# re-ovo/wgpu-path-tracing

Hardware: AMD Instinct MI355X
Metric: Msamples/s (rays x bounces / s) (higher is better)
Workload: dtype f32

## Files before the change

### wgpu-path-tracing_amd/csrc/pipeline.hip

```cpp
#include "pt_device.h"
#include "pt_math.h"

namespace {

constexpr int BLOCK = 256;

PT_DEV void camera_ray(const ptmi_camera &cam, uint32_t x, uint32_t y, uint32_t frame, v3 &org, v3 &dir,
                       uint32_t &rng) {
    rng = rng_seed(x, y, frame);
    float jx = rng_f(rng), jy = rng_f(rng);
    float px = (float)x + jx, py = (float)y + jy;
    float uvx = (px / (float)cam.width) * 2.0f - 1.0f;
    float uvy = (py / (float)cam.height) * 2.0f - 1.0f;
    float th = tan1(cam.fov * 0.5f);
    v3 fw = mk3(cam.forward[0], cam.forward[1], cam.forward[2]);
    v3 rt = mk3(cam.right[0], cam.right[1], cam.right[2]);
    v3 up = mk3(cam.up[0], cam.up[1], cam.up[2]);
    v3 pos = mk3(cam.position[0], cam.position[1], cam.position[2]);
    v3 a = scale3(scale3(scale3(rt, uvx), th), cam.aspect);
    v3 b = scale3(scale3(up, uvy), th);
    dir = normalize3(add3(add3(fw, a), b));
    org = pos;
    if (cam.aperture > 0.0f) {
        v3 focal = madd3(dir, cam.focus_distance, pos);
// ... 68 lines not shown
    __shared__ uint32_t wsum[TILE_WAVES], wssum[TILE_WAVES];
    const uint32_t count = *count_ptr;
    const uint32_t nwords = (count + 63u) >> 6;
    if (blockIdx.x == 0 && threadIdx.x == 0) {
        atomicAdd(&stats[0], (unsigned long long)count); atomicAdd(&stats[8 + bounce], (unsigned long long)count);
    }
    if (blockIdx.x * TILE_WORDS >= nwords) return;
    const uint32_t w = blockIdx.x * TILE_WORDS + threadIdx.x;
    uint32_t c = 0, sc = 0;
    if (w < nwords) { c = (uint32_t)__popcll(alive[w]); if (shadow) sc = (uint32_t)__popcll(shadow[w]); }
    for (int off = 32; off > 0; off >>= 1) { c += __shfl_down(c, off); sc += __shfl_down(sc, off); }
    if ((threadIdx.x & 63u) == 0u) { wsum[threadIdx.x >> 6] = c; wssum[threadIdx.x >> 6] = sc; }
    __syncthreads();
    if (threadIdx.x == 0) {
        uint32_t t = 0, ts = 0;
        for (int i = 0; i < TILE_WAVES; i++) { t += wsum[i]; ts += wssum[i]; }
        tile_sums[blockIdx.x] = t;
        shadow_tile_sums[blockIdx.x] = ts;
        if (ts) { atomicAdd(&stats[1], (unsigned long long)ts); atomicAdd(&stats[2], (unsigned long long)ts); }
    }
}

template <bool PACKED>
PT_DEV void scatter_tile(uint32_t tile, const uint32_t *__restrict__ count_ptr, const uint32_t *__restrict__ queue,
                         const uint64_t *__restrict__ alive, const uint32_t *__restrict__ tile_sums,
                         uint32_t *__restrict__ next_queue, uint32_t *__restrict__ next_count) {
    __shared__ uint32_t wtot[TILE_WAVES];
    __shared__ uint32_t tile_base;
    const uint32_t count = *count_ptr;
    const uint32_t nwords = (count + 63u) >> 6;
    const uint32_t ntiles = (nwords + TILE_WORDS - 1) / TILE_WORDS;
    if (tile >= ntiles) {
        if (ntiles == 0 && tile == 0 && threadIdx.x == 0) *next_count = 0;
        return;
    }
    const uint32_t lane = threadIdx.x & 63u, wave = threadIdx.x >> 6;
    uint32_t pre = 0;
    for (uint32_t t = threadIdx.x; t < tile; t += TILE_WORDS) pre += tile_sums[t];
    for (int off = 32; off > 0; off >>= 1) pre += __shfl_down(pre, off);
    if (lane == 0) wtot[wave] = pre;
    __syncthreads();
    if (threadIdx.x == 0) { uint32_t t = 0; for (int i = 0; i < TILE_WAVES; i++) t += wtot[i]; tile_base = t; }
    __syncthreads();
    const uint32_t base0 = tile_base;
    __syncthreads();
    const uint32_t w = tile * TILE_WORDS + threadIdx.x;
    const uint64_t m = w < nwords ? alive[w] : 0ull;
    const uint32_t c = (uint32_t)__popcll(m);
    uint32_t inc = c;
    for (int off = 1; off < 64; off <<= 1) { uint32_t v = __shfl_up(inc, off); if (lane >= (uint32_t)off) inc += v; }
    if (lane == 63u) wtot[wave] = inc;
    __syncthreads();
    uint32_t wbase = 0;
    for (uint32_t i = 0; i < wave; i++) wbase += wtot[i];
    const uint32_t my_off = base0 + wbase + inc - c;
    if (tile == ntiles - 1 && threadIdx.x == TILE_WORDS - 1) *next_count = my_off + c;
    const uint32_t mlo = (uint32_t)m, mhi = (uint32_t)(m >> 32);
    const uint32_t w0 = tile * TILE_WORDS + wave * 64u;
    for (uint32_t j = 0; j < 64u; j++) {
        const uint32_t jlo = __shfl(mlo, (int)j), jhi = __shfl(mhi, (int)j), jbase = __shfl(my_off, (int)j);
        const uint64_t jm = ((uint64_t)jhi << 32) | jlo;
        if (jm == 0ull) continue;
        if ((jm >> lane) & 1ull) {
            const uint32_t below = (uint32_t)__popcll(jm & ((1ull << lane) - 1ull));
            const uint32_t slot = (w0 + j) * 64u + lane;
            next_queue[jbase + below] = PACKED ? (w0 + j) * 64u + below : queue ? queue[slot] : slot;
        }
    }
}

__global__ __launch_bounds__(TILE_WORDS) void k_scatter(const uint32_t *__restrict__ count_ptr,
                                                        const uint32_t *__restrict__ queue,
                                                        const uint64_t *__restrict__ alive,
                                                        const uint32_t *__restrict__ tile_sums,
                                                        uint32_t *__restrict__ next_queue,
                                                        uint32_t *__restrict__ next_count) {
    scatter_tile<false>(blockIdx.x, count_ptr, queue, alive, tile_sums, next_queue, next_count);
}
__global__ __launch_bounds__(TILE_WORDS) void k_scatter_packed(const uint32_t *__restrict__ count_ptr,
                                                               const uint64_t *__restrict__ shadow,
                                                               const uint32_t *__restrict__ shadow_sums,
                                                               uint32_t *__restrict__ shadow_queue,
                                                               uint32_t *__restrict__ shadow_count) {
    scatter_tile<true>(blockIdx.x, count_ptr, nullptr, shadow, shadow_sums, shadow_queue, shadow_count);
}
__global__ __launch_bounds__(TILE_WORDS) void k_scatter2(uint32_t tiles, const uint32_t *__restrict__ count_ptr,
                                                         const uint32_t *__restrict__ queue,
                                                         const uint64_t *__restrict__ alive, const uint64_t *__restrict__ shadow,
                                                         const uint32_t *__restrict__ tile_sums, const uint32_t *__restrict__ shadow_sums,
                                                         uint32_t *__restrict__ next_queue, uint32_t *__restrict__ next_count,
                                                         uint32_t *__restrict__ shadow_queue, uint32_t *__restrict__ shadow_count) {
    if (blockIdx.x < tiles) scatter_tile<false>(blockIdx.x, count_ptr, queue, alive, tile_sums, next_queue, next_count);
    else scatter_tile<true>(blockIdx.x - tiles, count_ptr, nullptr, shadow, shadow_sums, shadow_queue, shadow_count);
}

__global__ __launch_bounds__(BLOCK) void k_repack(const uint32_t *__restrict__ count_ptr, const uint32_t *__restrict__ queue,
                                                  DevPaths from, DevPaths to, uint32_t *__restrict__ pid) {
    const uint32_t n = *count_ptr;
    for (uint32_t j = blockIdx.x * BLOCK + threadIdx.x; j < n; j += gridDim.x * BLOCK) {
        const uint32_t q = queue[j];
        const float4 o = ld_stream(&from.O[q]), d = ld_stream(&from.D[q]);
        const float2 c = ld_stream(&from.C[q]);
        st_stream(&to.O[j], o); st_stream(&to.D[j], d); st_stream(&to.C[j], c);
        pid[j] = q;
    }
}

template <int N>
PT_DEV void fold(float (&acc)[N], const float (&x)[N], uint32_t frame) {
    if (frame > 0u) {
        const float t = 1.0f / (float)(frame + 1u);
        for (int i = 0; i < N; i++) acc[i] = mix1(acc[i], x[i], t);
    } else {
        for (int i = 0; i < N; i++) acc[i] = x[i];
    }
}
PT_DEV rgb_sc ld_clamped(const float *__restrict__ L, uint32_t l_stride, size_t p) {
    rgb_sc l;
    if (l_stride == 4u) { const float4 v = reinterpret_cast<const float4 *>(L)[p]; l = rgb_sc{v.x, v.y, v.z}; }
    else l = reinterpret_cast<const rgb_sc *>(L)[p];
    return rgb_sc{min1(l.x, 2.5f), min1(l.y, 2.5f), min1(l.z, 2.5f)};
}

template <class Pixels>
PT_DEV void fold_radiance(const Pixels &px, uint32_t n_frames, const float *__restrict__ L, uint32_t l_stride, float4 *__restrict__ out) {
    const uint32_t n = px.entries();
    for (uint32_t j = blockIdx.x * BLOCK + threadIdx.x; j < n; j += gridDim.x * BLOCK) {
        const size_t oi = px.band.frame_pixel(px.pixel(j));
// ... 110 lines not shown
        const uint64_t word = __ballot(active);
        if ((threadIdx.x & 63u) == 0u) ballot[pix >> 6] = word;
    }
}

__global__ __launch_bounds__(TILE_WORDS) void k_ad_tile_sums(const uint32_t *__restrict__ count_ptr, const uint64_t *__restrict__ ballot,
                                                             uint32_t *__restrict__ tile_sums) {
    __shared__ uint32_t wsum[TILE_WAVES];
    const uint32_t nwords = (*count_ptr + 63u) >> 6;
    const uint32_t w = blockIdx.x * TILE_WORDS + threadIdx.x;
    uint32_t c = w < nwords ? (uint32_t)__popcll(ballot[w]) : 0u;
    for (int off = 32; off > 0; off >>= 1) c += __shfl_down(c, off);
    if ((threadIdx.x & 63u) == 0u) wsum[threadIdx.x >> 6] = c;
    __syncthreads();
    if (threadIdx.x == 0) {
        uint32_t t = 0;
        for (int i = 0; i < TILE_WAVES; i++) t += wsum[i];
        tile_sums[blockIdx.x] = t;
    }
}
__global__ __launch_bounds__(TILE_WORDS) void k_ad_scatter(const uint32_t *__restrict__ count_ptr, const uint64_t *__restrict__ ballot,
                                                           const uint32_t *__restrict__ tile_sums, uint32_t *__restrict__ list,
                                                           uint32_t *__restrict__ n_active) {
    scatter_tile<false>(blockIdx.x, count_ptr, nullptr, ballot, tile_sums, list, n_active);
}

__global__ __launch_bounds__(BLOCK) void k_ad_raygen(ptmi_camera cam, DevBand band, const uint32_t *__restrict__ list,
                                                     const uint32_t *__restrict__ n_active, uint32_t n_frames,
                                                     const float4 *__restrict__ mom, DevPaths P, uint32_t *__restrict__ count_out,
                                                     unsigned long long *__restrict__ traced) {
    if (blockIdx.x == 0 && threadIdx.x == 0) atomicAdd(&traced[0], (unsigned long long)(*n_active * n_frames));
    raygen(cam, ListedPixels{band, list, n_active, mom}, n_frames, P, count_out);
}
__global__ __launch_bounds__(BLOCK) void k_ad_accumulate(DevBand band, const uint32_t *__restrict__ list, const uint32_t *__restrict__ n_active,
                                                         uint32_t n_frames, const float4 *__restrict__ mom, const float *__restrict__ L,
                                                         uint32_t l_stride, float4 *__restrict__ out) {
    fold_radiance(ListedPixels{band, list, n_active, mom}, n_frames, L, l_stride, out);
}
__global__ __launch_bounds__(BLOCK) void k_ad_accumulate_aov(DevBand band, const uint32_t *__restrict__ list, const uint32_t *__restrict__ n_active,
                                                             uint32_t n_frames, const float4 *__restrict__ mom, const float4 *__restrict__ rec,
                                                             const ptmi_triangle *__restrict__ tris, uint32_t n_tris,
                                                             float4 *__restrict__ albedo, float4 *__restrict__ normal, uint2 *__restrict__ ids) {
    fold_aov(ListedPixels{band, list, n_active, mom}, n_frames, rec, tris, n_tris, albedo, normal, ids);
}
__global__ __launch_bounds__(BLOCK) void k_ad_accumulate_moments(DevBand band, const uint32_t *__restrict__ list,
                                                                 const uint32_t *__restrict__ n_active, uint32_t n_frames,
                                                                 const float *__restrict__ L, uint32_t l_stride, float4 *__restrict__ mom) {
// ... 98 lines not shown
        else if (which == 2) { if (__builtin_fabsf(x) < PT_EPS) continue; got = rcp1_above_eps(x); ref = 1.0f / x; }
        else { got = rcp1(x); ref = 1.0f / x; }
        if (__float_as_uint(got) != __float_as_uint(ref) && !(got != got && ref != ref)) { bad++; first = i < first ? i : first; }
    }
    if (bad) { atomicAdd(&out[0], bad); atomicMin(&out[1], first); }
}

}

void pt_launch_exact_math(hipStream_t s, int which, unsigned long long *out) {
    hipLaunchKernelGGL(k_exact_math, dim3(256 * 16), dim3(256), 0, s, which, out);
}
void pt_launch_raygen(hipStream_t s, int blocks, const ptmi_camera &cam, DevPixels px, uint32_t n_frames, DevPaths p,
                      uint32_t *count_out) {
    if (px.list)
        hipLaunchKernelGGL(k_ad_raygen, dim3(blocks), dim3(BLOCK), 0, s, cam, px.band, px.list, px.n_active, n_frames, px.mom, p, count_out,
                           px.traced);
    else hipLaunchKernelGGL(k_raygen, dim3(blocks), dim3(BLOCK), 0, s, cam, px.band, px.frame0, n_frames, p, count_out);
}
void pt_launch_raygen_list(hipStream_t s, const ptmi_camera &cam, uint32_t n, const uint32_t *xs,
                           const uint32_t *ys, const uint32_t *frames, DevPaths p) {
    hipLaunchKernelGGL(k_raygen_list, dim3((n + BLOCK - 1) / BLOCK), dim3(BLOCK), 0, s, cam, n, xs, ys, frames, p);
}
void pt_launch_compact(hipStream_t s, int tiles, const uint32_t *queue, const uint32_t *count,
                       const uint64_t *alive_mask, const uint64_t *shadow_mask, uint32_t *tile_sums,
                       uint32_t *next_queue, uint32_t *next_count, uint32_t *shadow_queue, uint32_t *shadow_count,
                       unsigned long long *stats, uint32_t bounce, int do_scatter) {
    uint32_t *shadow_sums = tile_sums + tiles;
    hipLaunchKernelGGL(k_tile_sums, dim3(tiles), dim3(TILE_WORDS), 0, s, count, alive_mask, shadow_mask, tile_sums,
                       shadow_sums, stats, bounce);
#ifndef PT_NO_SCATTER2
    if (do_scatter && shadow_mask) {
        hipLaunchKernelGGL(k_scatter2, dim3(2 * tiles), dim3(TILE_WORDS), 0, s, (uint32_t)tiles, count, queue, alive_mask, shadow_mask,
                           tile_sums, shadow_sums, next_queue, next_count, shadow_queue, shadow_count);
        return;
    }
#endif
    if (do_scatter)
        hipLaunchKernelGGL(k_scatter, dim3(tiles), dim3(TILE_WORDS), 0, s, count, queue, alive_mask, tile_sums,
                           next_queue, next_count);
    if (shadow_mask)
        hipLaunchKernelGGL(k_scatter_packed, dim3(tiles), dim3(TILE_WORDS), 0, s, count, shadow_mask, shadow_sums, shadow_queue,
                           shadow_count);
}
void pt_launch_repack(hipStream_t s, int blocks, const uint32_t *count, const uint32_t *queue, DevPaths from, DevPaths to,
                      uint32_t *pid) {
    hipLaunchKernelGGL(k_repack, dim3(blocks), dim3(BLOCK), 0, s, count, queue, from, to, pid);
}
void pt_launch_accumulate(hipStream_t s, int blocks, DevPixels px, uint32_t n_frames, const float *L, uint32_t l_stride, float4 *out) {
    if (px.list)
        hipLaunchKernelGGL(k_ad_accumulate, dim3(blocks), dim3(BLOCK), 0, s, px.band, px.list, px.n_active, n_frames, px.mom, L, l_stride, out);
    else hipLaunchKernelGGL(k_accumulate, dim3(blocks), dim3(BLOCK), 0, s, px.band, px.frame0, n_frames, L, l_stride, out);
}
void pt_launch_accumulate_aov(hipStream_t s, int blocks, DevPixels px, uint32_t n_frames, const float4 *rec,
                              const ptmi_triangle *tris, uint32_t n_tris, float4 *albedo, float4 *normal, uint2 *ids) {
    if (px.list)
        hipLaunchKernelGGL(k_ad_accumulate_aov, dim3(blocks), dim3(BLOCK), 0, s, px.band, px.list, px.n_active, n_frames, px.mom, rec, tris,
                           n_tris, albedo, normal, ids);
    else
        hipLaunchKernelGGL(k_accumulate_aov, dim3(blocks), dim3(BLOCK), 0, s, px.band, px.frame0, n_frames, rec, tris, n_tris, albedo, normal,
                           ids);
}
void pt_launch_accumulate_moments(hipStream_t s, int blocks, DevPixels px, uint32_t n_frames, const float *L, uint32_t l_stride,
                                  float4 *mom) {
    if (px.list)
        hipLaunchKernelGGL(k_ad_accumulate_moments, dim3(blocks), dim3(BLOCK), 0, s, px.band, px.list, px.n_active, n_frames, L, l_stride, mom);
    else hipLaunchKernelGGL(k_accumulate_moments, dim3(blocks), dim3(BLOCK), 0, s, px.band, px.frame0, n_frames, L, l_stride, mom);
}
void pt_launch_adaptive_restart(hipStream_t s, int blocks, DevBand band, float4 *mom) {
    hipLaunchKernelGGL(k_ad_restart, dim3(blocks), dim3(BLOCK), 0, s, band, mom);
// ... 28 lines not shown
```

### wgpu-path-tracing_amd/csrc/pt_device.h

```cpp
#pragma once
#include <hip/hip_runtime.h>
#include <stdint.h>
#include "ptmi_layout.h"
#include "ptmi.h"

#define PT_HD __host__ __device__ inline

#define PT_REF_LEAF      0x80000000u
#define PT_REF_NONE      0xFFFFFFFFu
#define PT_LEAF_MAX_TRIS 32u
#define PT_LEAF_OFF_BITS 26u
#define PT_LEAF_OFF_MASK ((1u << PT_LEAF_OFF_BITS) - 1u)

struct DevScene;
struct DevScene {
    const ptmi_triangle *tris;  uint32_t n_tris;
    const ptmi_material *mats;  uint32_t n_mats;
    const ptmi_light *lights;   uint32_t n_lights;
    const void *atlas;          uint32_t atlas_w, atlas_h, atlas_fmt;
    const float4 *wnodes;       uint32_t n_wnodes;
    const float4 *tripos;
    float root_min[3], root_max[3];
    uint32_t root_ref;
    const float4 *ref_wnodes;   uint32_t ref_root_ref, has_fast;
// ... 17 lines not shown
struct DevPaths {
    float4 *O, *D; float2 *C; float *L; uint32_t l_stride = 3;
    __device__ __forceinline__ rgb_sc ldL(uint32_t p) const {
        if (l_stride == 4u) { const float4 v = reinterpret_cast<const float4 *>(L)[p]; return rgb_sc{v.x, v.y, v.z}; }
        return reinterpret_cast<const rgb_sc *>(L)[p];
    }
    __device__ __forceinline__ void stL(uint32_t p, float x, float y, float z) const {
        if (l_stride == 4u) reinterpret_cast<float4 *>(L)[p] = make_float4(x, y, z, 0.0f);
        else reinterpret_cast<rgb_sc *>(L)[p] = rgb_sc{x, y, z};
    }
};
struct DevShadow { float4 *SO, *SD; rgb_sc *SC; uint32_t cap; };

struct DevBand {
    uint32_t width, height, y0, y1, strip, parts, part, rows;
    PT_HD uint32_t row_of(uint32_t l) const {
        if (parts <= 1u) return y0 + l;
        return y0 + ((l / strip) * parts + part) * strip + l % strip;
    }
    PT_HD size_t frame_pixel(uint32_t pix) const { return (size_t)row_of(pix / width) * width + pix % width; }
};

PT_HD bool pt_plays_roulette(uint32_t bounce) { return bounce > 2u; }
inline uint32_t pt_repack_bounce() { uint32_t b = 0; while (!pt_plays_roulette(b)) b++; return b; }

struct ShadeParams {
    uint32_t bounce, max_bounces, do_mis;
    unsigned long long *stats;
    uint32_t emit_records;
    const uint32_t *pid;
};

enum { PT_VARIANT_GLOBAL = 1, PT_VARIANT_LDS = 2, PT_VARIANT_LDS_NODES = 3,
       PT_VARIANT_OWN_LDS = 4, PT_VARIANT_OWN_LDS_NODES = 5, PT_VARIANT_OWN_QLDS = 6, PT_VARIANT_OWN_QLDS_NODES = 7,
       PT_VARIANT_OWN_QGLOBAL = 8, PT_VARIANT_OWN_GLOBAL = 9,
       PT_VARIANT_OWN_LDS16_NODES = 10,
       PT_VARIANT_OWN_QLDS16_NODES = 11,
       PT_VARIANT_COUNT };

enum PtNodes {
    PT_NODES_EXACT,
    PT_NODES_QUANT,
    PT_NODES_EXACT16,
    PT_NODES_QUANT16 };
enum PtWhere {
    PT_LDS_ALL,
    PT_LDS_NODES,
    PT_FROM_MEMORY };
enum PtStack {
    PT_STACK_DEPTH,
    PT_STACK_NODES,
    PT_STACK_SPILL,
    PT_STACK_16BIT,
// ... 47 lines not shown
    const uint32_t *list, *n_active; const float4 *mom;
    unsigned long long *traced;
};
void pt_launch_raygen(hipStream_t s, int blocks, const ptmi_camera &cam, DevPixels px, uint32_t n_frames, DevPaths p,
                      uint32_t *count_out);
void pt_launch_raygen_list(hipStream_t s, const ptmi_camera &cam, uint32_t n, const uint32_t *xs,
                           const uint32_t *ys, const uint32_t *frames, DevPaths p);
void pt_launch_extend(hipStream_t s, int blocks, const TraverseConfig &cfg, const DevScene &sc, DevPaths p,
                      const uint32_t *queue, const uint32_t *count, float2 *hits);
void pt_launch_extend_own(hipStream_t s, int blocks, const TraverseConfig &cfg, const DevScene &sc, DevPaths p,
                          const uint32_t *queue, const uint32_t *count, float2 *hits);
void pt_launch_hit_uv(hipStream_t s, uint32_t n, const DevScene &sc, DevPaths p, const float2 *hits, float2 *uv);
void pt_launch_shadow(hipStream_t s, int blocks, const TraverseConfig &cfg, const DevScene &sc, DevPaths p,
                      DevShadow sh, const uint32_t *shadow_queue, const uint32_t *count, uint8_t *occluded_out);
void pt_launch_shadow_own(hipStream_t s, int blocks, const TraverseConfig &cfg, const DevScene &sc, DevPaths p,
                          DevShadow sh, const uint32_t *shadow_queue, const uint32_t *count, uint8_t *occluded_out);
void pt_launch_shade(hipStream_t s, int blocks, const DevScene &sc, DevPaths p, const uint32_t *queue,
                     const uint32_t *count, const float2 *hits, DevShadow sh, uint64_t *alive_mask,
                     uint64_t *shadow_mask, ShadeParams sp, float4 *aov = nullptr);
void pt_launch_shade_fast(hipStream_t s, int blocks, const DevScene &sc, DevPaths p, const uint32_t *queue,
                          const uint32_t *count, const float2 *hits, DevShadow sh, uint64_t *alive_mask,
                          uint64_t *shadow_mask, ShadeParams sp, float4 *aov = nullptr);
uint32_t pt_compact_tile_slots(void);
void pt_launch_repack(hipStream_t s, int blocks, const uint32_t *count, const uint32_t *queue, DevPaths from, DevPaths to,
                      uint32_t *pid);
void pt_launch_compact(hipStream_t s, int tiles, const uint32_t *queue, const uint32_t *count,
                       const uint64_t *alive_mask, const uint64_t *shadow_mask, uint32_t *tile_sums,
                       uint32_t *next_queue, uint32_t *next_count, uint32_t *shadow_queue, uint32_t *shadow_count,
                       unsigned long long *stats, uint32_t bounce, int do_scatter);
void pt_launch_accumulate(hipStream_t s, int blocks, DevPixels px, uint32_t n_frames, const float *L, uint32_t l_stride, float4 *out);
void pt_launch_accumulate_aov(hipStream_t s, int blocks, DevPixels px, uint32_t n_frames, const float4 *rec,
                              const ptmi_triangle *tris, uint32_t n_tris, float4 *albedo, float4 *normal, uint2 *ids);
void pt_launch_accumulate_moments(hipStream_t s, int blocks, DevPixels px, uint32_t n_frames, const float *L, uint32_t l_stride,
                                  float4 *mom);
struct DevAdaptive {
    uint64_t *ballot;
    uint32_t *list;
    uint32_t *tile_sums;
    uint32_t *ctl;
    unsigned long long *acc;
};
uint32_t pt_adaptive_tiles(uint32_t npix);
void pt_launch_adaptive_restart(hipStream_t s, int blocks, DevBand band, float4 *mom);
void pt_launch_adaptive_list(hipStream_t s, int blocks, DevBand band, const ptmi_adaptive_params &ap, const float4 *mom, DevAdaptive ad);
void pt_launch_adaptive_status(hipStream_t s, int blocks, DevBand band, const float4 *mom, DevAdaptive ad);
struct DenoiseArgs {
    uint32_t W, H, iterations;
    float phi_color, phi_normal, phi_depth;
};
// ... 23 lines not shown
```

### wgpu-path-tracing_amd/csrc/ptmi_api.hip

```cpp
#include "ptmi.h"
#include "pt_device.h"
#include "fast_tree.h"

#include <algorithm>
#include <chrono>
#include <cmath>
#include <cstdarg>
#include <cstdint>
#include <cstdio>
#include <cstring>
#include <deque>
#include <memory>
#include <string>
#include <typeinfo>
#include <utility>
#include <vector>

namespace {

thread_local std::string g_create_err;

enum SceneBuf {
    kTris, kMats, kLights,
    kRefWnodes, kRefTripos,
    kWnodes, kTripos,
    kQnodes, kLeafStream,
    kLeafbox,
    kWnodes16, kRefWnodes16, kQnodes16,
    kSceneBufs
};

struct EventPair { hipEvent_t a, b; int kind; };
constexpr size_t kMaxPendingEvents = 4096;

}

struct Lane {
    size_t cap = 0;
    DevPaths paths{};
    float2 *hits = nullptr;
    DevShadow sh[2]{};
    uint32_t *queue[2] = {nullptr, nullptr}, *sq[2] = {nullptr, nullptr};
    DevPaths tail{};
    uint32_t *pid = nullptr;
    uint64_t *alive = nullptr, *shadowm = nullptr;
    size_t mask_words = 0;
    uint32_t *word_off = nullptr, *counts = nullptr;
    uint32_t *d_spill = nullptr;
    uint32_t *d_spill_side = nullptr;
    uint8_t *d_occ = nullptr;
    hipStream_t side = nullptr;
    hipEvent_t ev_ready = nullptr, ev_shadow[2] = {nullptr, nullptr};
    float4 *aov = nullptr;
};

struct ptmi_ctx {
    int device = 0, n_cu = 256;
    hipStream_t own_stream = nullptr, stream = nullptr;
    Lane lane;
    mutable std::string err;
    bool alloc_oom = false;
    ptmi_options opt{};

    void *buf[kSceneBufs] = {};
    void *d_atlas = nullptr;
    DevScene *d_scene = nullptr;
    DevScene sc{};
// ... 97 lines not shown
        c->event_pool.push_back(c->in_flight.front()); c->in_flight.pop_front();
    }
    return hipSuccess;
}

struct Timed {
    ptmi_ctx *c; hipEvent_t a = nullptr, b = nullptr; int kind; bool on;
    hipStream_t st;
    Timed(ptmi_ctx *c_, int kind_, bool on_, hipStream_t st_ = nullptr) : c(c_), kind(kind_), on(on_), st(st_ ? st_ : c_->stream) {
        if (on) { a = get_event(c); b = get_event(c); (void)hipEventRecord(a, st); }
    }
    ~Timed() {
        if (!on) return;
        (void)hipEventRecord(b, st);
        c->pending.push_back({a, b, kind});
        if (c->pending.size() > kMaxPendingEvents) drain_completed_events(c);
    }
};

void free_batch(Lane &ln) {
    dfree(ln.paths.O); dfree(ln.paths.D); dfree(ln.paths.C); dfree(ln.paths.L);
    dfree(ln.hits);
    for (int k = 0; k < 2; k++) { dfree(ln.sh[k].SO); ln.sh[k].SD = nullptr; ln.sh[k].SC = nullptr; dfree(ln.sq[k]); }
    dfree(ln.tail.O); dfree(ln.tail.D); dfree(ln.tail.C); dfree(ln.pid);
    dfree(ln.queue[0]); dfree(ln.queue[1]); dfree(ln.alive); dfree(ln.shadowm); dfree(ln.word_off); dfree(ln.d_occ);
    dfree(ln.aov);
    ln.cap = 0;
}

hipError_t sync_all(ptmi_ctx *c) {
    hipError_t e = c->stream ? hipStreamSynchronize(c->stream) : hipSuccess;
    if (e == hipSuccess && c->lane.side) e = hipStreamSynchronize(c->lane.side);
    if (e == hipSuccess && c->stream) e = hipStreamSynchronize(c->stream);
    return e;
}

constexpr size_t kBytesPerPath = 16 + 16 + 8 + 16 + 8 + 2 * (16 + 16 + sizeof(rgb_sc) + 4) + (16 + 16 + 8 + 4) + 2 * 4 + 1 + 1;
#ifndef PT_REPACK
#define PT_REPACK 1
#endif
constexpr size_t kAovBytesPerPath = 32;
size_t bytes_per_path(bool aov) { return kBytesPerPath + (aov ? kAovBytesPerPath : 0); }

int ensure_capacity(ptmi_ctx *c, Lane &ln, size_t n) {
    const bool aov = c->aov_mask != 0;
    if (n <= ln.cap && (!aov || ln.aov)) return PTMI_OK;
    HIP_TRY(c, sync_all(c));
    free_batch(ln);
    size_t cap = (n + 1023) & ~(size_t)1023;
    size_t words = cap / 64 + 1;
    size_t tiles = cap / pt_compact_tile_slots() + 2;
    c->alloc_oom = false;
#define ALLOC(ptr, bytes) do { hipError_t e_ = hipMalloc(&(ptr), (bytes)); if (e_ != hipSuccess) { \
        c->alloc_oom = e_ == hipErrorOutOfMemory; free_batch(ln); (void)hipGetLastError(); \
        return fail(c, PTMI_E_HIP, "hipMalloc of %zu bytes for a batch of %zu paths failed: %s", (size_t)(bytes), cap, hipGetErrorString(e_)); } } while (0)
    ALLOC(ln.paths.O, cap * 16); ALLOC(ln.paths.D, cap * 16);
    ALLOC(ln.paths.C, cap * 8); ALLOC(ln.paths.L, cap * 16);
    ALLOC(ln.hits, cap * 8);
    for (int k = 0; k < 2; k++) {
        ALLOC(ln.sh[k].SO, cap * (16 + 16 + sizeof(rgb_sc)));
        ln.sh[k].SD = ln.sh[k].SO + cap; ln.sh[k].SC = reinterpret_cast<rgb_sc *>(ln.sh[k].SO + 2 * cap); ln.sh[k].cap = (uint32_t)cap;
        ALLOC(ln.sq[k], cap * 4);
    }
    ALLOC(ln.tail.O, cap * 16); ALLOC(ln.tail.D, cap * 16); ALLOC(ln.tail.C, cap * 8); ALLOC(ln.pid, cap * 4);
    ALLOC(ln.queue[0], cap * 4); ALLOC(ln.queue[1], cap * 4);
    ALLOC(ln.alive, words * 8); ALLOC(ln.shadowm, words * 8); ln.mask_words = words;
    ALLOC(ln.word_off, 2 * tiles * 4);
    ALLOC(ln.d_occ, cap);
    if (aov) ALLOC(ln.aov, cap * kAovBytesPerPath);
#undef ALLOC
    ln.cap = cap;
    return PTMI_OK;
}

struct HeldBuf {
    bool present = false;
    std::shared_ptr<const void> keep;
    const std::type_info *type = nullptr;
    const void *host = nullptr;
    void *dev = nullptr;
    int device = -1;
    size_t bytes = 0;
};

struct Built {
    HeldBuf buf[kSceneBufs];
    ptmi_image_info img{};
// ... 794 lines not shown
    if (cfg_shadow0.wants_spill && !ln.d_spill_side) HIP_TRY(c, hipMalloc(&ln.d_spill_side, pt_spill_bytes(c->n_cu * 8)));
    c->st.traversal_used = pt_variant(cfg0.variant).where == PT_FROM_MEMORY ? PTMI_TRAVERSAL_GLOBAL : PTMI_TRAVERSAL_LDS;
    c->st.extend_variant = pt_variant_code(cfg0);
    c->st.shadow_variant = pt_variant_code(cfg_shadow0);
    c->st.frames_per_batch_used = F;
    c->st.radiance_stride_bytes = (walks_memory_quantised(cfg0) || walks_memory_quantised(cfg_shadow0)) ? 16u : 12u;
    const int blocks = c->n_cu * 8;
#ifndef PT_SHADE_WGS_PER_CU
#define PT_SHADE_WGS_PER_CU 16
#endif
    const int shade_blocks = c->n_cu * PT_SHADE_WGS_PER_CU;
    const uint32_t maxb = c->opt.max_bounces;
    const bool t1 = c->opt.timing >= 1, t2 = c->opt.timing >= 2, t3 = c->opt.timing >= 3;
    {
        Timed td(c, 0, t1);
        const hipStream_t ms = c->stream;
        const hipStream_t ss = side ? ln.side : ms;
        const int tiles = (int)(ln.cap / pt_compact_tile_slots() + 1);
        TraverseConfig cfg = cfg0, cfg_shadow = cfg_shadow0;
        cfg.spill = ln.d_spill; cfg_shadow.spill = side ? ln.d_spill_side : ln.d_spill;
        if (cfg_shadow.wants_spill && !cfg_shadow.spill) cfg_shadow.spill = ln.d_spill_side;
        ln.paths.l_stride = c->st.radiance_stride_bytes / 4u;
        const DevPaths bp = ln.paths;
        const uint32_t rb = PT_REPACK ? pt_repack_bounce() : 0xFFFFFFFEu;
        DevPaths tp = ln.tail;
        tp.L = bp.L; tp.l_stride = bp.l_stride;
        float4 *const aov_rec = c->aov_mask ? ln.aov : nullptr;
        if (ap && cam->frame_index == 0u) { pt_launch_adaptive_restart(ms, blocks, band, c->d_moments); c->ad_rounds = 0; }
        auto batch = [&](uint32_t frame0, uint32_t fb) -> int {
            const DevPixels px = ap ? DevPixels{band, 0u, c->ad.list, &c->ad.ctl[1], c->d_moments, c->ad.acc}
                                    : DevPixels{band, frame0, nullptr, nullptr, nullptr, nullptr};
            { Timed t(c, 4, t3, ms); pt_launch_raygen(ms, blocks, *cam, px, fb, bp, &ln.counts[0]); }
            int cur = 0;
            for (uint32_t b = 0; b < maxb; b++) {
                const bool tail = b > rb;
                const uint32_t *q = b == 0 || b == rb + 1 ? nullptr : ln.queue[cur];
                const DevPaths sp = tail ? tp : bp;
                const int par = side ? (int)(b & 1u) : 0;
                const ShadeParams shp{b, maxb, c->opt.do_mis, c->d_stats, side ? 1u : 0u, tail ? ln.pid : nullptr};
                { Timed t(c, 1, t2, ms); (c->sc.own ? pt_launch_extend_own : pt_launch_extend)(ms, blocks, cfg, c->sc, sp, q, &ln.counts[b], ln.hits); }
                const bool last = b + 1 == maxb;
                if (side && b >= 2) HIP_TRY(c, hipStreamWaitEvent(ms, ln.ev_shadow[par], 0));
                { Timed t(c, 2, t3, ms);
                  (c->opt.perf_mode ? pt_launch_shade_fast : pt_launch_shade)(
                      ms, shade_blocks, c->sc, sp, q, &ln.counts[b], ln.hits, ln.sh[par], ln.alive, ln.shadowm, shp,
                      b == 0 ? aov_rec : nullptr); }
                { Timed t(c, 5, t3, ms);
                  pt_launch_compact(ms, tiles, q, &ln.counts[b], ln.alive, nee ? ln.shadowm : nullptr,
                                    ln.word_off, ln.queue[cur ^ 1], &ln.counts[b + 1], ln.sq[par], &ln.counts[kShadowCount + par],
                                    c->d_stats, b, last ? 0 : 1);
                  if (b == rb && !last) pt_launch_repack(ms, blocks, &ln.counts[b + 1], ln.queue[cur ^ 1], bp, tp, ln.pid); }
                if (side) {
                    HIP_TRY(c, hipEventRecord(ln.ev_ready, ms));
                    HIP_TRY(c, hipStreamWaitEvent(ss, ln.ev_ready, 0));
                    { Timed t(c, 3, t3, ss);
                      (c->sc.own ? pt_launch_shadow_own : pt_launch_shadow)(ss, blocks, cfg_shadow, c->sc, bp, ln.sh[par], ln.sq[par],
                                                                            &ln.counts[kShadowCount + par], nullptr); }
                    HIP_TRY(c, hipEventRecord(ln.ev_shadow[par], ss));
                } else if (nee) {
                    Timed t(c, 3, t3, ms);
                    (c->sc.own ? pt_launch_shadow_own : pt_launch_shadow)(ms, blocks, cfg_shadow, c->sc, bp, ln.sh[0], ln.sq[0], &ln.counts[kShadowCount], nullptr);
                }
                cur ^= 1;
            }
            if (side) {
                HIP_TRY(c, hipStreamWaitEvent(ms, ln.ev_shadow[(maxb - 1) & 1u], 0));
                if (maxb >= 2) HIP_TRY(c, hipStreamWaitEvent(ms, ln.ev_shadow[maxb & 1u], 0));
            }
            Timed t(c, 6, t3, ms);
            pt_launch_accumulate(ms, blocks, px, fb, bp.L, bp.l_stride, c->d_out);
            if (aov_rec)
                pt_launch_accumulate_aov(ms, blocks, px, fb, aov_rec, c->sc.tris, c->sc.n_tris, c->d_aov_albedo, c->d_aov_normal,
                                         c->d_aov_id);
            if (ap || c->d_moments) pt_launch_accumulate_moments(ms, blocks, px, fb, bp.L, bp.l_stride, c->d_moments);
// ... 576 lines not shown
```

### wgpu-path-tracing_amd/csrc/shade.hip

```cpp
#include "pt_device.h"
#include "pt_math.h"

namespace {

struct HitInfo {
    v3 position; float t;
    v3 normal;
    v3 albedo;
    float roughness, metallic, transmission, ior;
    v3 emission; float emissive_strength;
    bool is_front;
};

PT_DEV v3 ld3(const float *p) { return mk3(p[0], p[1], p[2]); }

PT_DEV v4 atlas_load(const DevScene &sc, uint32_t x, uint32_t y) {
    v4 r; r.x = r.y = r.z = r.w = 0.0f;
    if (sc.atlas_fmt == 0u || x >= sc.atlas_w || y >= sc.atlas_h) return r;
    size_t idx = ((size_t)y * sc.atlas_w + x);
    if (sc.atlas_fmt == 1u) {
        const uint2 raw = reinterpret_cast<const uint2 *>(sc.atlas)[idx];
        union { uint32_t u; _Float16 h[2]; } a, b;
        a.u = raw.x; b.u = raw.y;
        r.x = (float)a.h[0]; r.y = (float)a.h[1]; r.z = (float)b.h[0]; r.w = (float)b.h[1];
// ... 226 lines not shown
#define PT_SHADE_WAVES 0
#endif
#if PT_SHADE_WAVES > 0
#define PT_SHADE_ATTR __attribute__((amdgpu_waves_per_eu(PT_SHADE_WAVES)))
#else
#define PT_SHADE_ATTR
#endif

template <bool AOV>
__global__ __launch_bounds__(SBLOCK) PT_SHADE_ATTR void k_shade(DevScene sc, DevPaths P, const uint32_t *__restrict__ queue,
                                                  const uint32_t *__restrict__ count_ptr,
                                                  const float2 *__restrict__ hits, DevShadow S,
                                                  uint64_t *__restrict__ alive_mask,
                                                  uint64_t *__restrict__ shadow_mask, ShadeParams sp,
                                                  float4 *__restrict__ aov) {
    const uint32_t count = *count_ptr;
    const uint32_t lane = threadIdx.x & 63u;
    uint32_t n_skipped = 0, n_emitted = 0;
    for (uint32_t base = blockIdx.x * SBLOCK; base < count; base += gridDim.x * SBLOCK) {
        const uint32_t i = base + threadIdx.x;
        bool alive = false, shadow = false, skipped = false, emitted = false;
        float4 rec_o = make_float4(0.0f, 0.0f, 0.0f, -2.0f), rec_d = make_float4(0.0f, 0.0f, 0.0f, 0.0f);
        rgb_sc rec_c{0.0f, 0.0f, 0.0f};
        if (i < count) {
            const uint32_t q = queue ? queue[i] : i;
            const float2 h2 = ld_stream(&hits[i]);
            if (!(h2.x < 0.0f)) {
                const float4 o4 = ld_stream(&P.O[q]), d4 = ld_stream(&P.D[q]);
                const uint32_t p = sp.pid ? sp.pid[q] : q;
                uint32_t rng = __float_as_uint(o4.w);
                const v3 ro = xyz(o4), rd = xyz(d4);
                v3 thr = mk3(1.0f, 1.0f, 1.0f);
                if (sp.bounce != 0u) { const float2 c2 = ld_stream(&P.C[q]); thr = mk3(d4.w, c2.x, c2.y); }
                const HitInfo hit = make_hitinfo(sc, ro, rd, h2.x, __float_as_uint(h2.y));
                if (AOV) {
                    st_stream(&aov[2 * (size_t)i], make_float4(hit.albedo.x, hit.albedo.y, hit.albedo.z, hit.t));
                    st_stream(&aov[2 * (size_t)i + 1], make_float4(hit.normal.x, hit.normal.y, hit.normal.z, h2.y));
                }
                if (hit.emission.x > 0.0f || hit.emission.y > 0.0f || hit.emission.z > 0.0f) {
                    float att = rcp1(1.0f + hit.t * hit.t);
                    float k = hit.emissive_strength;
                    const v3 e = mk3(thr.x * hit.emission.x * k * att, thr.y * hit.emission.y * k * att, thr.z * hit.emission.z * k * att);
                    if (sp.emit_records) {
                        rec_d.w = __uint_as_float(p);
                        rec_c = rgb_sc{e.x, e.y, e.z};
                        shadow = true; emitted = true;
// ... 16 lines not shown
                                rec_o = make_float4(so.x, so.y, so.z, ls.dist);
                                rec_d = make_float4(ls.wi.x, ls.wi.y, ls.wi.z, __uint_as_float(p));
                                rec_c = rgb_sc{contrib.x, contrib.y, contrib.z};
                                shadow = true;
                            } else {
                                skipped = true;
                            }
                        } else if (ls.traced) {
                            skipped = true;
                        }
                    }
                    v3 dir = sample_bsdf(rng, hit, rd, hit.is_front);
                    v4 ev = eval_bsdf(hit, hit.normal, neg3(normalize3(rd)), dir, hit.is_front);
                    if (!(ev.w <= 0.0f)) {
                        v3 no = madd3(dir, PT_EPS, hit.position);
                        v3 nd = normalize3(dir);
                        thr = mul3(thr, vdiv3(mk3(ev.x, ev.y, ev.z), max1(ev.w, PT_EPS)));
                        alive = true;
                        if (pt_plays_roulette(sp.bounce)) {
                            float pr = max1(max1(thr.x, thr.y), thr.z);
                            if (rng_f(rng) > pr) alive = false;
                            else thr = vdiv3(thr, pr);
                        }
                        if (alive && sp.bounce + 1u < sp.max_bounces) {
                            st_stream(&P.O[q], make_float4(no.x, no.y, no.z, __uint_as_float(rng)));
                            st_stream(&P.D[q], make_float4(nd.x, nd.y, nd.z, thr.x));
                            st_stream(&P.C[q], make_float2(thr.y, thr.z));
                        }
                    }
                }
            } else if (AOV) {
                st_stream(&aov[2 * (size_t)i], make_float4(0.0f, 0.0f, 0.0f, 0.0f));
                st_stream(&aov[2 * (size_t)i + 1], make_float4(0.0f, 0.0f, 0.0f, __uint_as_float(0xFFFFFFFFu)));
            } else if (sp.bounce != 0u) {
                const float tx = reinterpret_cast<const float *>(&P.D[q])[3];
                const float2 c2 = ld_stream(&P.C[q]);
                if (!(__builtin_isfinite(tx) & __builtin_isfinite(c2.x) & __builtin_isfinite(c2.y))) {
                    const uint32_t p = sp.pid ? sp.pid[q] : q;
                    const v3 e = mk3(tx * 0.0f, c2.x * 0.0f, c2.y * 0.0f);
                    if (sp.emit_records) {
                        rec_d.w = __uint_as_float(p);
                        rec_c = rgb_sc{e.x, e.y, e.z};
                        shadow = true; emitted = true;
                    } else {
                        const rgb_sc l = P.ldL(p);
                        P.stL(p, l.x + e.x, l.y + e.y, l.z + e.z);
                    }
                }
            }
        }
        const uint64_t am = __ballot(alive), sm = __ballot(shadow), zm = __ballot(skipped), em = __ballot(emitted);
        if (shadow) {
            const uint32_t r = (i & ~63u) + (uint32_t)__popcll(sm & ((1ull << lane) - 1ull));
            st_stream(&S.SO[r], rec_o);
            st_stream(&S.SD[r], rec_d);
            S.SC[r] = rec_c;
        }
        if (lane == 0u && i < count) {
            alive_mask[i >> 6] = am;
            shadow_mask[i >> 6] = sm;
            n_skipped += (uint32_t)__popcll(zm);
            n_emitted += (uint32_t)__popcll(em);
        }
    }
    if (n_skipped) atomicAdd(&sp.stats[1], (unsigned long long)n_skipped);
    if (n_emitted) atomicAdd(&sp.stats[3], (unsigned long long)n_emitted);
}

}

#ifdef PT_SHADE_FAST
#define PT_LAUNCH_SHADE pt_launch_shade_fast
#else
#define PT_LAUNCH_SHADE pt_launch_shade
// ... 32 lines not shown
```

Measured before the change: 11260.

## Write surviving paths compacted into ping-pong buffers instead of indirect queue plus repack

Shade now writes each surviving path's next-bounce state into a second path buffer at a wave-compacted slot (using the alive ballot), along with its pixel id. Scatter becomes a packed word-offset map for both alive and shadow lists. The separate repack kernel and the queue indirection are removed, so every bounce reads a nearly contiguous path set. This costs a second full path buffer and pid array, and the next bounce goes through the packed list into the partner buffer.

```diff
diff --git a/wgpu-path-tracing_amd/csrc/pipeline.hip b/wgpu-path-tracing_amd/csrc/pipeline.hip
--- a/wgpu-path-tracing_amd/csrc/pipeline.hip
+++ b/wgpu-path-tracing_amd/csrc/pipeline.hip
@@ -114,8 +114,7 @@
 }
 
 template <bool PACKED>
-PT_DEV void scatter_tile(uint32_t tile, const uint32_t *__restrict__ count_ptr, const uint32_t *__restrict__ queue,
-                         const uint64_t *__restrict__ alive, const uint32_t *__restrict__ tile_sums,
+PT_DEV void scatter_tile(uint32_t tile, const uint32_t *__restrict__ count_ptr, const uint64_t *__restrict__ alive, const uint32_t *__restrict__ tile_sums,
                          uint32_t *__restrict__ next_queue, uint32_t *__restrict__ next_count) {
     __shared__ uint32_t wtot[TILE_WAVES];
     __shared__ uint32_t tile_base;
@@ -155,47 +154,25 @@
         if (jm == 0ull) continue;
         if ((jm >> lane) & 1ull) {
             const uint32_t below = (uint32_t)__popcll(jm & ((1ull << lane) - 1ull));
-            const uint32_t slot = (w0 + j) * 64u + lane;
-            next_queue[jbase + below] = PACKED ? (w0 + j) * 64u + below : queue ? queue[slot] : slot;
+            next_queue[jbase + below] = (w0 + j) * 64u + (PACKED ? below : lane);
         }
     }
 }
 
 __global__ __launch_bounds__(TILE_WORDS) void k_scatter(const uint32_t *__restrict__ count_ptr,
-                                                        const uint32_t *__restrict__ queue,
-                                                        const uint64_t *__restrict__ alive,
+                                                        const uint64_t *__restrict__ mask,
                                                         const uint32_t *__restrict__ tile_sums,
-                                                        uint32_t *__restrict__ next_queue,
-                                                        uint32_t *__restrict__ next_count) {
-    scatter_tile<false>(blockIdx.x, count_ptr, queue, alive, tile_sums, next_queue, next_count);
-}
-__global__ __launch_bounds__(TILE_WORDS) void k_scatter_packed(const uint32_t *__restrict__ count_ptr,
-                                                               const uint64_t *__restrict__ shadow,
-                                                               const uint32_t *__restrict__ shadow_sums,
-                                                               uint32_t *__restrict__ shadow_queue,
-                                                               uint32_t *__restrict__ shadow_count) {
-    scatter_tile<true>(blockIdx.x, count_ptr, nullptr, shadow, shadow_sums, shadow_queue, shadow_count);
+                                                        uint32_t *__restrict__ list,
+                                                        uint32_t *__restrict__ list_count) {
+    scatter_tile<true>(blockIdx.x, count_ptr, mask, tile_sums, list, list_count);
 }
 __global__ __launch_bounds__(TILE_WORDS) void k_scatter2(uint32_t tiles, const uint32_t *__restrict__ count_ptr,
-                                                         const uint32_t *__restrict__ queue,
                                                          const uint64_t *__restrict__ alive, const uint64_t *__restrict__ shadow,
                                                          const uint32_t *__restrict__ tile_sums, const uint32_t *__restrict__ shadow_sums,
                                                          uint32_t *__restrict__ next_queue, uint32_t *__restrict__ next_count,
                                                          uint32_t *__restrict__ shadow_queue, uint32_t *__restrict__ shadow_count) {
-    if (blockIdx.x < tiles) scatter_tile<false>(blockIdx.x, count_ptr, queue, alive, tile_sums, next_queue, next_count);
-    else scatter_tile<true>(blockIdx.x - tiles, count_ptr, nullptr, shadow, shadow_sums, shadow_queue, shadow_count);
-}
-
-__global__ __launch_bounds__(BLOCK) void k_repack(const uint32_t *__restrict__ count_ptr, const uint32_t *__restrict__ queue,
-                                                  DevPaths from, DevPaths to, uint32_t *__restrict__ pid) {
-    const uint32_t n = *count_ptr;
-    for (uint32_t j = blockIdx.x * BLOCK + threadIdx.x; j < n; j += gridDim.x * BLOCK) {
-        const uint32_t q = queue[j];
-        const float4 o = ld_stream(&from.O[q]), d = ld_stream(&from.D[q]);
-        const float2 c = ld_stream(&from.C[q]);
-        st_stream(&to.O[j], o); st_stream(&to.D[j], d); st_stream(&to.C[j], c);
-        pid[j] = q;
-    }
+    if (blockIdx.x < tiles) scatter_tile<true>(blockIdx.x, count_ptr, alive, tile_sums, next_queue, next_count);
+    else scatter_tile<true>(blockIdx.x - tiles, count_ptr, shadow, shadow_sums, shadow_queue, shadow_count);
 }
 
 template <int N>
@@ -352,7 +329,7 @@
 __global__ __launch_bounds__(TILE_WORDS) void k_ad_scatter(const uint32_t *__restrict__ count_ptr, const uint64_t *__restrict__ ballot,
                                                            const uint32_t *__restrict__ tile_sums, uint32_t *__restrict__ list,
                                                            uint32_t *__restrict__ n_active) {
-    scatter_tile<false>(blockIdx.x, count_ptr, nullptr, ballot, tile_sums, list, n_active);
+    scatter_tile<false>(blockIdx.x, count_ptr, ballot, tile_sums, list, n_active);
 }
 
 __global__ __launch_bounds__(BLOCK) void k_ad_raygen(ptmi_camera cam, DevBand band, const uint32_t *__restrict__ list,
@@ -497,7 +474,7 @@
                            const uint32_t *ys, const uint32_t *frames, DevPaths p) {
     hipLaunchKernelGGL(k_raygen_list, dim3((n + BLOCK - 1) / BLOCK), dim3(BLOCK), 0, s, cam, n, xs, ys, frames, p);
 }
-void pt_launch_compact(hipStream_t s, int tiles, const uint32_t *queue, const uint32_t *count,
+void pt_launch_compact(hipStream_t s, int tiles, const uint32_t *count,
                        const uint64_t *alive_mask, const uint64_t *shadow_mask, uint32_t *tile_sums,
                        uint32_t *next_queue, uint32_t *next_count, uint32_t *shadow_queue, uint32_t *shadow_count,
                        unsigned long long *stats, uint32_t bounce, int do_scatter) {
@@ -506,21 +483,17 @@
                        shadow_sums, stats, bounce);
 #ifndef PT_NO_SCATTER2
     if (do_scatter && shadow_mask) {
-        hipLaunchKernelGGL(k_scatter2, dim3(2 * tiles), dim3(TILE_WORDS), 0, s, (uint32_t)tiles, count, queue, alive_mask, shadow_mask,
+        hipLaunchKernelGGL(k_scatter2, dim3(2 * tiles), dim3(TILE_WORDS), 0, s, (uint32_t)tiles, count, alive_mask, shadow_mask,
                            tile_sums, shadow_sums, next_queue, next_count, shadow_queue, shadow_count);
         return;
     }
 #endif
     if (do_scatter)
-        hipLaunchKernelGGL(k_scatter, dim3(tiles), dim3(TILE_WORDS), 0, s, count, queue, alive_mask, tile_sums,
+        hipLaunchKernelGGL(k_scatter, dim3(tiles), dim3(TILE_WORDS), 0, s, count, alive_mask, tile_sums,
                            next_queue, next_count);
     if (shadow_mask)
-        hipLaunchKernelGGL(k_scatter_packed, dim3(tiles), dim3(TILE_WORDS), 0, s, count, shadow_mask, shadow_sums, shadow_queue,
+        hipLaunchKernelGGL(k_scatter, dim3(tiles), dim3(TILE_WORDS), 0, s, count, shadow_mask, shadow_sums, shadow_queue,
                            shadow_count);
-}
-void pt_launch_repack(hipStream_t s, int blocks, const uint32_t *count, const uint32_t *queue, DevPaths from, DevPaths to,
-                      uint32_t *pid) {
-    hipLaunchKernelGGL(k_repack, dim3(blocks), dim3(BLOCK), 0, s, count, queue, from, to, pid);
 }
 void pt_launch_accumulate(hipStream_t s, int blocks, DevPixels px, uint32_t n_frames, const float *L, uint32_t l_stride, float4 *out) {
     if (px.list)
diff --git a/wgpu-path-tracing_amd/csrc/pt_device.h b/wgpu-path-tracing_amd/csrc/pt_device.h
--- a/wgpu-path-tracing_amd/csrc/pt_device.h
+++ b/wgpu-path-tracing_amd/csrc/pt_device.h
@@ -63,13 +63,14 @@
 };
 
 PT_HD bool pt_plays_roulette(uint32_t bounce) { return bounce > 2u; }
-inline uint32_t pt_repack_bounce() { uint32_t b = 0; while (!pt_plays_roulette(b)) b++; return b; }
 
 struct ShadeParams {
     uint32_t bounce, max_bounces, do_mis;
     unsigned long long *stats;
     uint32_t emit_records;
     const uint32_t *pid;
+    DevPaths next;
+    uint32_t *next_pid;
 };
 
 enum { PT_VARIANT_GLOBAL = 1, PT_VARIANT_LDS = 2, PT_VARIANT_LDS_NODES = 3,
@@ -163,9 +164,7 @@
                           const uint32_t *count, const float2 *hits, DevShadow sh, uint64_t *alive_mask,
                           uint64_t *shadow_mask, ShadeParams sp, float4 *aov = nullptr);
 uint32_t pt_compact_tile_slots(void);
-void pt_launch_repack(hipStream_t s, int blocks, const uint32_t *count, const uint32_t *queue, DevPaths from, DevPaths to,
-                      uint32_t *pid);
-void pt_launch_compact(hipStream_t s, int tiles, const uint32_t *queue, const uint32_t *count,
+void pt_launch_compact(hipStream_t s, int tiles, const uint32_t *count,
                        const uint64_t *alive_mask, const uint64_t *shadow_mask, uint32_t *tile_sums,
                        uint32_t *next_queue, uint32_t *next_count, uint32_t *shadow_queue, uint32_t *shadow_count,
                        unsigned long long *stats, uint32_t bounce, int do_scatter);
diff --git a/wgpu-path-tracing_amd/csrc/ptmi_api.hip b/wgpu-path-tracing_amd/csrc/ptmi_api.hip
--- a/wgpu-path-tracing_amd/csrc/ptmi_api.hip
+++ b/wgpu-path-tracing_amd/csrc/ptmi_api.hip
@@ -41,8 +41,8 @@
     float2 *hits = nullptr;
     DevShadow sh[2]{};
     uint32_t *queue[2] = {nullptr, nullptr}, *sq[2] = {nullptr, nullptr};
-    DevPaths tail{};
-    uint32_t *pid = nullptr;
+    DevPaths paths1{};
+    uint32_t *pid[2] = {nullptr, nullptr};
     uint64_t *alive = nullptr, *shadowm = nullptr;
     size_t mask_words = 0;
     uint32_t *word_off = nullptr, *counts = nullptr;
@@ -186,7 +186,7 @@
     dfree(ln.paths.O); dfree(ln.paths.D); dfree(ln.paths.C); dfree(ln.paths.L);
     dfree(ln.hits);
     for (int k = 0; k < 2; k++) { dfree(ln.sh[k].SO); ln.sh[k].SD = nullptr; ln.sh[k].SC = nullptr; dfree(ln.sq[k]); }
-    dfree(ln.tail.O); dfree(ln.tail.D); dfree(ln.tail.C); dfree(ln.pid);
+    dfree(ln.paths1.O); dfree(ln.paths1.D); dfree(ln.paths1.C); dfree(ln.pid[0]); dfree(ln.pid[1]);
     dfree(ln.queue[0]); dfree(ln.queue[1]); dfree(ln.alive); dfree(ln.shadowm); dfree(ln.word_off); dfree(ln.d_occ);
     dfree(ln.aov);
     ln.cap = 0;
@@ -199,10 +199,7 @@
     return e;
 }
 
-constexpr size_t kBytesPerPath = 16 + 16 + 8 + 16 + 8 + 2 * (16 + 16 + sizeof(rgb_sc) + 4) + (16 + 16 + 8 + 4) + 2 * 4 + 1 + 1;
-#ifndef PT_REPACK
-#define PT_REPACK 1
-#endif
+constexpr size_t kBytesPerPath = 16 + 16 + 8 + 16 + 8 + 2 * (16 + 16 + sizeof(rgb_sc) + 4) + (16 + 16 + 8) + 2 * 4 + 2 * 4 + 1 + 1;
 constexpr size_t kAovBytesPerPath = 32;
 size_t bytes_per_path(bool aov) { return kBytesPerPath + (aov ? kAovBytesPerPath : 0); }
 
@@ -226,7 +223,8 @@
         ln.sh[k].SD = ln.sh[k].SO + cap; ln.sh[k].SC = reinterpret_cast<rgb_sc *>(ln.sh[k].SO + 2 * cap); ln.sh[k].cap = (uint32_t)cap;
         ALLOC(ln.sq[k], cap * 4);
     }
-    ALLOC(ln.tail.O, cap * 16); ALLOC(ln.tail.D, cap * 16); ALLOC(ln.tail.C, cap * 8); ALLOC(ln.pid, cap * 4);
+    ALLOC(ln.paths1.O, cap * 16); ALLOC(ln.paths1.D, cap * 16); ALLOC(ln.paths1.C, cap * 8);
+    ALLOC(ln.pid[0], cap * 4); ALLOC(ln.pid[1], cap * 4);
     ALLOC(ln.queue[0], cap * 4); ALLOC(ln.queue[1], cap * 4);
     ALLOC(ln.alive, words * 8); ALLOC(ln.shadowm, words * 8); ln.mask_words = words;
     ALLOC(ln.word_off, 2 * tiles * 4);
@@ -1067,9 +1065,8 @@
         if (cfg_shadow.wants_spill && !cfg_shadow.spill) cfg_shadow.spill = ln.d_spill_side;
         ln.paths.l_stride = c->st.radiance_stride_bytes / 4u;
         const DevPaths bp = ln.paths;
-        const uint32_t rb = PT_REPACK ? pt_repack_bounce() : 0xFFFFFFFEu;
-        DevPaths tp = ln.tail;
-        tp.L = bp.L; tp.l_stride = bp.l_stride;
+        DevPaths set[2] = {bp, ln.paths1};
+        set[1].L = bp.L; set[1].l_stride = bp.l_stride;
         float4 *const aov_rec = c->aov_mask ? ln.aov : nullptr;
         if (ap && cam->frame_index == 0u) { pt_launch_adaptive_restart(ms, blocks, band, c->d_moments); c->ad_rounds = 0; }
         auto batch = [&](uint32_t frame0, uint32_t fb) -> int {
@@ -1078,11 +1075,11 @@
             { Timed t(c, 4, t3, ms); pt_launch_raygen(ms, blocks, *cam, px, fb, bp, &ln.counts[0]); }
             int cur = 0;
             for (uint32_t b = 0; b < maxb; b++) {
-                const bool tail = b > rb;
-                const uint32_t *q = b == 0 || b == rb + 1 ? nullptr : ln.queue[cur];
-                const DevPaths sp = tail ? tp : bp;
+                const uint32_t *q = b == 0 ? nullptr : ln.queue[cur];
+                const DevPaths sp = set[cur];
                 const int par = side ? (int)(b & 1u) : 0;
-                const ShadeParams shp{b, maxb, c->opt.do_mis, c->d_stats, side ? 1u : 0u, tail ? ln.pid : nullptr};
+                const ShadeParams shp{b, maxb, c->opt.do_mis, c->d_stats, side ? 1u : 0u, b == 0 ? nullptr : ln.pid[cur],
+                                      set[cur ^ 1], ln.pid[cur ^ 1]};
                 { Timed t(c, 1, t2, ms); (c->sc.own ? pt_launch_extend_own : pt_launch_extend)(ms, blocks, cfg, c->sc, sp, q, &ln.counts[b], ln.hits); }
                 const bool last = b + 1 == maxb;
                 if (side && b >= 2) HIP_TRY(c, hipStreamWaitEvent(ms, ln.ev_shadow[par], 0));
@@ -1091,10 +1088,9 @@
                       ms, shade_blocks, c->sc, sp, q, &ln.counts[b], ln.hits, ln.sh[par], ln.alive, ln.shadowm, shp,
                       b == 0 ? aov_rec : nullptr); }
                 { Timed t(c, 5, t3, ms);
-                  pt_launch_compact(ms, tiles, q, &ln.counts[b], ln.alive, nee ? ln.shadowm : nullptr,
+                  pt_launch_compact(ms, tiles, &ln.counts[b], ln.alive, nee ? ln.shadowm : nullptr,
                                     ln.word_off, ln.queue[cur ^ 1], &ln.counts[b + 1], ln.sq[par], &ln.counts[kShadowCount + par],
-                                    c->d_stats, b, last ? 0 : 1);
-                  if (b == rb && !last) pt_launch_repack(ms, blocks, &ln.counts[b + 1], ln.queue[cur ^ 1], bp, tp, ln.pid); }
+                                    c->d_stats, b, last ? 0 : 1); }
                 if (side) {
                     HIP_TRY(c, hipEventRecord(ln.ev_ready, ms));
                     HIP_TRY(c, hipStreamWaitEvent(ss, ln.ev_ready, 0));
diff --git a/wgpu-path-tracing_amd/csrc/shade.hip b/wgpu-path-tracing_amd/csrc/shade.hip
--- a/wgpu-path-tracing_amd/csrc/shade.hip
+++ b/wgpu-path-tracing_amd/csrc/shade.hip
@@ -272,6 +272,9 @@
         bool alive = false, shadow = false, skipped = false, emitted = false;
         float4 rec_o = make_float4(0.0f, 0.0f, 0.0f, -2.0f), rec_d = make_float4(0.0f, 0.0f, 0.0f, 0.0f);
         rgb_sc rec_c{0.0f, 0.0f, 0.0f};
+        float4 nxt_o = make_float4(0.0f, 0.0f, 0.0f, 0.0f), nxt_d = nxt_o;
+        float2 nxt_c = make_float2(0.0f, 0.0f);
+        uint32_t nxt_p = 0u;
         if (i < count) {
             const uint32_t q = queue ? queue[i] : i;
             const float2 h2 = ld_stream(&hits[i]);
@@ -334,11 +337,10 @@
                             if (rng_f(rng) > pr) alive = false;
                             else thr = vdiv3(thr, pr);
                         }
-                        if (alive && sp.bounce + 1u < sp.max_bounces) {
-                            st_stream(&P.O[q], make_float4(no.x, no.y, no.z, __uint_as_float(rng)));
-                            st_stream(&P.D[q], make_float4(nd.x, nd.y, nd.z, thr.x));
-                            st_stream(&P.C[q], make_float2(thr.y, thr.z));
-                        }
+                        nxt_o = make_float4(no.x, no.y, no.z, __uint_as_float(rng));
+                        nxt_d = make_float4(nd.x, nd.y, nd.z, thr.x);
+                        nxt_c = make_float2(thr.y, thr.z);
+                        nxt_p = p;
                     }
                 }
             } else if (AOV) {
@@ -362,6 +364,13 @@
             }
         }
         const uint64_t am = __ballot(alive), sm = __ballot(shadow), zm = __ballot(skipped), em = __ballot(emitted);
+        if (alive && sp.bounce + 1u < sp.max_bounces) {
+            const uint32_t r = (i & ~63u) + (uint32_t)__popcll(am & ((1ull << lane) - 1ull));
+            st_stream(&sp.next.O[r], nxt_o);
+            st_stream(&sp.next.D[r], nxt_d);
+            st_stream(&sp.next.C[r], nxt_c);
+            sp.next_pid[r] = nxt_p;
+        }
         if (shadow) {
             const uint32_t r = (i & ~63u) + (uint32_t)__popcll(sm & ((1ull << lane) - 1ull));
             st_stream(&S.SO[r], rec_o);
```

After: 11840 (median of 6 runs). +5.2%, better.
